# alexv879/ClusterMachineLearningForHospitalNetworks-Apache-Spark

Hardware: AMD Instinct MI355X
Metric: KMeans fit samples/sec (whole node), 100M×256 k=256 at 1/2/4/8 MI355X (higher is better)
Workload: dtype bf16; 1 GPU; model=KMeans k=256, 100000000x256, global_batch=100000000, parallelism=dp1, k=256, rows=100000000, dim=256

## Files before the change

clustermachinelearningforhospitalnetworks_apache_spark_amd/_native/csrc/kmeans.hip:

```cpp
#include <algorithm>

#include "common.h"

namespace {

constexpr int kAccumThreads = 1024;
constexpr int kSegThreads = 256;

template <int DP>
struct AssignShape {
  static constexpr int NCH = DP / 8;
  static constexpr int KS = DP >= 32 ? DP / 32 : 1;
};
constexpr int kAssignThreads = 512;

template <bool HI>
__device__ __forceinline__ unsigned f8x2_to_bf16x2(unsigned w) {
  typedef float f2 __attribute__((ext_vector_type(2)));
  const f2 v = __builtin_amdgcn_cvt_pk_f32_fp8((int)w, HI);
  return (__float_as_uint(v.x) >> 16) | (__float_as_uint(v.y) & 0xffff0000u);
}

template <int DP, bool F8>
__device__ __forceinline__ void load_x16(const void* __restrict__ Xv, long long n, long long ldx, long long row0,
// ... 1432 lines not shown
                        hist, rank, dout, rr::Ext{}, grid, g_rr_dbg, st);
  }
  if (xfp8) {
    switch (Dp) {
#define CML_ASSIGN8(DP)                                                                                          \
  case DP:                                                                                                       \
    return launch_assign<DP, true>(X, n, ldx, c, ldc, kc, kp, c_base, cnorm, xnorm, labels, best, first, last,  \
                                   cost_part, hist, rank, dout, grid, st)
      CML_ASSIGN8(64); CML_ASSIGN8(128); CML_ASSIGN8(256); CML_ASSIGN8(512);
#undef CML_ASSIGN8
      default: return (int)hipErrorInvalidValue;
    }
  }
#define CML_ASSIGN(DS, DP)                                                                                       \
  case DS:                                                                                                       \
    return launch_assign<DP, false>(X, n, ldx, c, ldc, kc, kp, c_base, cnorm, xnorm, labels, best, first, last, \
                                    cost_part, hist, rank, dout, grid, st)
  switch (Dp / 16) {
    CML_ASSIGN(1, 16); CML_ASSIGN(2, 32); CML_ASSIGN(4, 64); CML_ASSIGN(8, 128); CML_ASSIGN(16, 256);
    CML_ASSIGN(32, 512);
    default: return (int)hipErrorInvalidValue;
  }
#undef CML_ASSIGN
}

CML_API int cml_kmeans_assign_rr_ext(int mode, const void* X, long long n, long long ldx, int Dp, const void* C,
                                     long long ldc, int kc, int kp, const float* cnorm, const float* xnorm,
                                     int* labels, double* cost_part, int* hist, int* rank, int grid, int xfp8,
                                     int* chg_rows, int* chg_old, int* chg_wg_count, int* chg_overflow, int chg_pcap,
                                     int rr_ct, const int* idx, const int* n_dev, const int* lab_in, float* ub,
                                     float* lb, const float* mc, float tau, const int* gate, int want, float* best,
                                     const float* cum, int k_cum, float* mcost, int* mnear, int moff,
                                     void* stream) {
  if (mode < 1 || mode > 2 || kc != kp || kc % 16 != 0 || ldc % 8 != 0) return (int)hipErrorInvalidValue;
  if ((mcost == nullptr) != (mnear == nullptr) || (mcost != nullptr && mode != 2)) return (int)hipErrorInvalidValue;
  if (xfp8 ? (ldx % 16 != 0) : (ldx % 8 != 0)) return (int)hipErrorInvalidValue;
  if (rr_ct <= 0 || rr::plan_ct(Dp, kc, xfp8 != 0) != rr_ct) return (int)hipErrorInvalidValue;
  if (xnorm == nullptr || ub == nullptr || lb == nullptr || mc == nullptr) return (int)hipErrorInvalidValue;
  if ((hist == nullptr) != (rank == nullptr)) return (int)hipErrorInvalidValue;
  if (mode == 2 && (idx == nullptr || n_dev == nullptr || lab_in == nullptr || hist != nullptr))
    return (int)hipErrorInvalidValue;
  if (chg_rows != nullptr && (chg_old == nullptr || chg_wg_count == nullptr || chg_overflow == nullptr || chg_pcap < 0))
    return (int)hipErrorInvalidValue;
  const long long lds = rr::lds_for(Dp, kp, xfp8 != 0, mode);
  if (lds <= 0 || lds > 160 * 1024) return (int)hipErrorInvalidValue;
  const DeltaOut dout{chg_rows, chg_old, chg_wg_count, chg_overflow, chg_pcap, nullptr};
  const rr::Ext ext{idx,  n_dev, lab_in, ub,    lb,    mc,   tau, gate, want, cum, cum != nullptr ? cum + k_cum : nullptr,
                    mcost, mnear, moff};
  return rr::dispatch(mode, Dp, rr_ct, xfp8 != 0, X, n, ldx, (const u16*)C, ldc, kc, kp, cnorm, xnorm, labels,
                      best, cost_part, hist, rank, dout, ext, grid, g_rr_dbg, (hipStream_t)stream);
}

extern "C" int cml_kmeans_row_pass(const void* X, long long n, long long ldx, int Dp, int xfp8, float* xn,
                                   const float* c0, float c0n, float* cost, int* near, unsigned* xn_max,
                                   int* erange, double* xn64, const float* c0n_dev, void* stream);

CML_API int cml_row_sqnorm_fp8(const void* X, long long n, long long ldx, int Dp, float* out, void* stream) {
  return cml_kmeans_row_pass(X, n, ldx, Dp, 1, out, nullptr, 0.f, nullptr, nullptr, nullptr, nullptr, nullptr,
                             nullptr, stream);
}

CML_API int cml_row_sqnorm_bf16(const void* X, long long n, long long ldx, int Dp, float* out, void* stream) {
  return cml_kmeans_row_pass(X, n, ldx, Dp, 0, out, nullptr, 0.f, nullptr, nullptr, nullptr, nullptr, nullptr,
                             nullptr, stream);
}

CML_API long long cml_kmeans_priv_lds_bytes(int k, int dw, int rpw) { return priv_lds_bytes(k, dw, rpw); }

CML_API int cml_kmeans_accum_priv(const void* X, long long n, long long ldx, const int* labels, int k, int dw, int cpl,
                                  int rpw, float* slab, int* cslab, int gx, int nsl, void* stream) {
  hipStream_t st = (hipStream_t)stream;
// ... 174 lines not shown
```

clustermachinelearningforhospitalnetworks_apache_spark_amd/_native/csrc/kmeans_rr.h:

```cpp
#pragma once

namespace rr {

constexpr int kThreads = 512;
constexpr int kCompute = 4;

struct Ext {
  const int* idx;
  const int* n_dev;
  const int* lab_in;
  float* ub;
  float* lb;
  const float* mc;
  float tau;
  const int* gate;
  int want;
  const float* cu = nullptr;
  const float* cl = nullptr;
  float* mcost = nullptr;
  int* mnear = nullptr;
  int moff = 0;
};

__host__ __device__ constexpr int cn_slots(int kp) { return ((kp + 3) & ~3) > 256 ? ((kp + 3) & ~3) : 256; }

template <int DP, bool F8 = false, int MODE = 0, bool M32 = false>
struct Geo {
  static constexpr int KS = DP / 32;
  static constexpr int ROWB = F8 ? DP : DP * 2;
  static constexpr int TR = 32768 / ROWB;
  static constexpr int NSUB = TR / 16;
  static constexpr int SLOT = TR * ROWB;
  static constexpr int PIECES = SLOT / 1024;
  static constexpr int RPP = 1024 / ROWB;
  static constexpr int LPR = ROWB / 16;
  static constexpr int TRAIL_Q = TR >= 64 ? TR / 64 : 1;
  static constexpr int NARR = MODE == 2 ? 3 : 2;
  static constexpr int CNT0 = PIECES / 2 + TRAIL_Q;
  static constexpr int CNT1 = PIECES / 2 + (NARR - 1) * TRAIL_Q;
  static constexpr int TRB = TR * 4 * NARR;
  static constexpr int NK = MODE >= 1 ? 2 : 1;
  static constexpr int NQ = M32 ? 8 : 16;
  static constexpr int STRIDE = NQ * NK + 1;
  static constexpr int RED = TR * STRIDE * 4;
  static constexpr int LAG = M32 ? 2 : 1;
  static constexpr int NKB = LAG + 1;
  static constexpr long long fixed_bytes(int ns, int kp) {
    const long long kp4 = (kp + 3) & ~3;
    return (long long)(ns + LAG) * TRB + (long long)NKB * RED + 4LL * kp4 + (M32 ? 4LL * cn_slots(kp) : 0LL) + 64;
  }
  static constexpr int NS = (4LL * SLOT + fixed_bytes(4, 1024)) <= 160 * 1024 ? 4 : 3;
  static constexpr int NTR = NS + LAG;
};

template <int DP, bool F8 = false, int MODE = 0, bool M32 = false>
__host__ __device__ constexpr long long lds_bytes(int kp) {
  using G = Geo<DP, F8, MODE, M32>;
  return (long long)G::NS * G::SLOT + G::fixed_bytes(G::NS, kp);
}

template <int N>
__device__ __forceinline__ void wait_vm() {
  static_assert(N >= 0 && N < 64, "vmcnt field is 6 bits");
  __builtin_amdgcn_s_waitcnt((N & 15) | ((N >> 4) << 14) | (7 << 4) | (15 << 8));
}

__device__ __forceinline__ void wait_lgkm0() { asm volatile("s_waitcnt lgkmcnt(0)" ::: "memory"); }

__device__ __forceinline__ void barrier() {
  asm volatile("" ::: "memory");
  __builtin_amdgcn_s_barrier();
  asm volatile("" ::: "memory");
}

__device__ __forceinline__ void glds16(const void* src, unsigned char* lds) {
  __builtin_amdgcn_global_load_lds(src, (__attribute__((address_space(3))) void*)lds, 16, 0, 0);
}
__device__ __forceinline__ void glds4(const void* src, unsigned char* lds) {
  __builtin_amdgcn_global_load_lds(src, (__attribute__((address_space(3))) void*)lds, 4, 0, 0);
}

typedef const __attribute__((address_space(4))) int* cidx_t;

__device__ __forceinline__ int med3(int a, int b, int c) {
  const int lo = a < b ? a : b, hi = a < b ? b : a;
// ... 316 lines not shown
        }
        sc2[h] = mx_split_half(w0, w1, wh[h], wl[h]);
        __builtin_amdgcn_sched_barrier(0);
      }
      chi[ct][b] = mx_v8i{(int)wh[0][0], (int)wh[0][1], (int)wh[0][2], (int)wh[0][3],
                          (int)wh[1][0], (int)wh[1][1], (int)wh[1][2], (int)wh[1][3]};
      clo[ct][b] = mx_v8i{(int)wl[0][0], (int)wl[0][1], (int)wl[0][2], (int)wl[0][3],
                          (int)wl[1][0], (int)wl[1][1], (int)wl[1][2], (int)wl[1][3]};
      const int src = r + 16 * (2 * (g & 1));
      const int s0 = __shfl(sc2[0], src, 64);
      const int s1 = __shfl(sc2[1], src, 64);
      csc[ct][b] = (g >> 1) ? s1 : s0;
      __builtin_amdgcn_sched_barrier(0);
    }
#pragma unroll
    for (int i = 0; i < 4; ++i) {
      const int c2 = cw0 + ct * 16 + 4 * g + i;
      c4[ct][i] = c2 < kc ? cnorm[c2] : __builtin_huge_valf();
    }
  }
  __builtin_amdgcn_s_setprio(1);
  int boff[4];
#pragma unroll
  for (int b = 0; b < 4; ++b) boff[b] = r * G::ROWB + (((4 * b + g) ^ r) << 4);
  barrier();
  for (long long j = 0; j < nt; ++j) {
    if (dbg & 2) {
      wait_lgkm0();
      barrier();
      continue;
    }
    const unsigned char* xs = smem + (int)(j % G::NS) * G::SLOT;
    const float* tn = reinterpret_cast<const float*>(trail + (int)(j % G::NTR) * G::TRB);
    int* kred = red + (int)(j & 1) * G::TR * G::STRIDE;
    float xnv[G::NSUB];
#pragma unroll
    for (int t = 0; t < G::NSUB; ++t) xnv[t] = tn[16 * t + r];
    auto xaddr = [&](int u) {
      const int t = u / UPS, v = u % UPS;
      return xs + 16 * t * G::ROWB + 256 * (v >> 2) + boff[v & 3];
    };
    uint4 xr[RING];
#pragma unroll
    for (int u = 0; u < PF && u < NU; ++u) xr[u] = *reinterpret_cast<const uint4*>(xaddr(u));
    f32x4 acc[2][CT];
    int key[2] = {0x7fffffff, 0x7fffffff};
    int key2[2] = {0x7fffffff, 0x7fffffff};
#pragma unroll
    for (int u = 0; u < NU; ++u) {
      const int t = u / UPS, v = u % UPS, cur = t & 1, prv = cur ^ 1;
      if (u + PF < NU) xr[(u + PF) % RING] = *reinterpret_cast<const uint4*>(xaddr(u + PF));
      if (v & 1) {
        const int s = v >> 1;
        const uint4 a0 = xr[(u - 1) % RING], a1 = xr[u % RING];
        const mx_v8i xb = mx_v8i{(int)a0.x, (int)a0.y, (int)a0.z, (int)a0.w, (int)a1.x, (int)a1.y, (int)a1.z, (int)a1.w};
        if (s == 0) {
          key[cur] = 0x7fffffff;
          if constexpr (TOP2) key2[cur] = 0x7fffffff;
        }
#pragma unroll
        for (int ct = 0; ct < CT; ++ct) {
          const f32x4 a = __builtin_amdgcn_mfma_scale_f32_16x16x128_f8f6f4(
              chi[ct][s], xb, s == 0 ? (c4[ct] + xnv[t]) : acc[cur][ct], 0, 0, 0, csc[ct][s], 0, 127);
          acc[cur][ct] = __builtin_amdgcn_mfma_scale_f32_16x16x128_f8f6f4(clo[ct][s], xb, a, 0, 0, 1, csc[ct][s], 0, 127);
        }
        if (t > 0) {
#pragma unroll
          for (int e = (s * CT * 4) / NB; e < ((s + 1) * CT * 4) / NB; ++e) {
            const int ct = e >> 2, i = e & 3;
            const int kv = (__float_as_int(acc[prv][ct][i]) & ~TAGM) | (ct << 2 | i);
            if constexpr (TOP2) key2[prv] = med3(key[prv], kv, key2[prv]);
            key[prv] = kv < key[prv] ? kv : key[prv];
          }
          if (s == NB - 1) {
            kred[(16 * (t - 1) + r) * G::STRIDE + wave * 4 + g] = key[prv];
            if constexpr (TOP2) kred[(16 * (t - 1) + r) * G::STRIDE + 16 + wave * 4 + g] = key2[prv];
          }
        }
      }
      __builtin_amdgcn_sched_barrier(0);
    }
    {
      constexpr int t = G::NSUB - 1, cur = t & 1;
#pragma unroll
      for (int e = 0; e < CT * 4; ++e) {
        const int ct = e >> 2, i = e & 3;
        const int kv = (__float_as_int(acc[cur][ct][i]) & ~TAGM) | (ct << 2 | i);
        if constexpr (TOP2) key2[cur] = med3(key[cur], kv, key2[cur]);
        key[cur] = kv < key[cur] ? kv : key[cur];
      }
      kred[(16 * t + r) * G::STRIDE + wave * 4 + g] = key[cur];
      if constexpr (TOP2) kred[(16 * t + r) * G::STRIDE + 16 + wave * 4 + g] = key2[cur];
    }
    wait_lgkm0();
    barrier();
  }
}

template <int DP, int CT, bool F8, int MODE, bool M32, bool MX = false>
__global__ __launch_bounds__(kThreads, 1) void kmeans_assign_rr(
    const unsigned char* __restrict__ X, long long n, long long ldx, const u16* __restrict__ C, long long ldc, int kc,
    int kp, const float* __restrict__ cnorm, const float* __restrict__ xnorm, int* __restrict__ labels,
    float* __restrict__ best_out, double* __restrict__ cost_part, int* __restrict__ hist_out,
    int* __restrict__ rank_out, DeltaOut dout, Ext ext, int dbg) {
  using G = Geo<DP, F8, MODE, M32>;
  constexpr int KS = G::KS;
  constexpr int NS = G::NS;
  constexpr int CPW = CT * 16;
  constexpr int TAGB = 2 + (CT > 1) + (CT > 2) + (CT > 4);
  constexpr int TAGM = (1 << TAGB) - 1;
  constexpr bool TOP2 = MODE >= 1;
  if (ext.gate != nullptr && *ext.gate != ext.want) return;
  if constexpr (MODE == 2) n = *ext.n_dev;
  const int* lab_src = MODE == 2 ? ext.lab_in : labels;
  extern __shared__ __attribute__((aligned(16))) unsigned char smem[];
  unsigned char* trail = smem + NS * G::SLOT;
  int* red = reinterpret_cast<int*>(trail + G::NTR * G::TRB);
  int* hist = red + G::NKB * G::TR * G::STRIDE;
  float* cnl = reinterpret_cast<float*>(hist + ((kp + 3) & ~3));
  int* misc = M32 ? reinterpret_cast<int*>(cnl + cn_slots(kp)) : hist + ((kp + 3) & ~3);
  double* cost_sh = reinterpret_cast<double*>(misc + 2);

  const int tid = threadIdx.x, lane = tid & 63, wave = __builtin_amdgcn_readfirstlane(tid >> 6);
  const long long ntiles = (n + G::TR - 1) / G::TR;
  const long long nt = ntiles > blockIdx.x ? (ntiles - 1 - blockIdx.x) / gridDim.x + 1 : 0;
  const bool ranking = rank_out != nullptr;
  auto tile_of = [&](long long j) { return (long long)blockIdx.x + j * gridDim.x; };

  if (wave < kCompute) {
// ... 2 lines not shown
   } else if constexpr (M32) {
    for (int i = tid; i < cn_slots(kp); i += kCompute * 64) cnl[i] = i < kc ? cnorm[i] : __builtin_huge_valf();
    compute_m32<DP, CT, F8, MODE>(C, ldc, kc, nt, wave, lane, smem, cnl, dbg);
   } else {
    const int r = lane & 15, g = lane >> 4;
    const int cw0 = wave * CPW;
    bf16x8 creg[CT][KS];
    f32x4 c4[CT];
#pragma unroll
    for (int ct = 0; ct < CT; ++ct) {
      const int c = cw0 + ct * 16 + r;
#pragma unroll
      for (int s = 0; s < KS; ++s) {
        uint4 v = make_uint4(0u, 0u, 0u, 0u);
        const int k0 = F8 ? 64 * (s >> 1) + 16 * g + 8 * (s & 1) : 32 * s + 8 * g;
        if (c < kc) v = *reinterpret_cast<const uint4*>(C + (long long)c * ldc + k0);
        const unsigned w4[4] = {v.x, v.y, v.z, v.w};
        unsigned o[4];
#pragma unroll
        for (int e = 0; e < 4; ++e) {
          const float lo = -2.f * bf16_to_f32((u16)(w4[e] & 0xffffu));
          const float hi = -2.f * bf16_to_f32((u16)(w4[e] >> 16));
          o[e] = (unsigned)f32_to_bf16(lo) | ((unsigned)f32_to_bf16(hi) << 16);
        }
        creg[ct][s] = __builtin_bit_cast(bf16x8, make_uint4(o[0], o[1], o[2], o[3]));
      }
#pragma unroll
      for (int i = 0; i < 4; ++i) {
        const int c2 = cw0 + ct * 16 + 4 * g + i;
        c4[ct][i] = c2 < kc ? cnorm[c2] : __builtin_huge_valf();
      }
    }
    __builtin_amdgcn_s_setprio(1);
    int boff[4];
#pragma unroll
    for (int b = 0; b < 4; ++b) boff[b] = r * G::ROWB + (((4 * b + g) ^ r) << 4);
    barrier();
    for (long long j = 0; j < nt; ++j) {
      if (dbg & 2) {
        wait_lgkm0();
        barrier();
        continue;
      }
      const unsigned char* xs = smem + (int)(j % NS) * G::SLOT;
      const float* tn = reinterpret_cast<const float*>(trail + (int)(j % G::NTR) * G::TRB);
      int* kred = red + (int)(j & 1) * G::TR * G::STRIDE;
      constexpr int SPU = F8 ? 2 : 1;
      constexpr int UPS = KS / SPU;
      constexpr int NU = G::NSUB * UPS;
      constexpr int PF = 3;
      float xnv[G::NSUB];
#pragma unroll
      for (int t = 0; t < G::NSUB; ++t) xnv[t] = tn[16 * t + r];
      auto xaddr = [&](int u) {
        const int t = u / UPS, v = u % UPS;
        return xs + 16 * t * G::ROWB + 256 * (v >> 2) + boff[v & 3];
      };
      uint4 xr[PF + 1];
#pragma unroll
      for (int u = 0; u < PF && u < NU; ++u) xr[u] = *reinterpret_cast<const uint4*>(xaddr(u));
      f32x4 acc[2][CT];
      int key[2] = {0x7fffffff, 0x7fffffff};
      int key2[2] = {0x7fffffff, 0x7fffffff};
#pragma unroll
      for (int u = 0; u < NU; ++u) {
        const int t = u / UPS, v = u % UPS, cur = t & 1, prv = cur ^ 1;
        if (u + PF < NU) xr[(u + PF) % (PF + 1)] = *reinterpret_cast<const uint4*>(xaddr(u + PF));
        bf16x8 xb[SPU];
        if constexpr (F8) {
          const uint4 w = xr[u % (PF + 1)];
          const unsigned ws[4] = {w.x, w.y, w.z, w.w};
          unsigned o[8];
#pragma unroll
          for (int q = 0; q < 4; ++q) {
            o[2 * q] = __builtin_bit_cast(unsigned, __builtin_amdgcn_cvt_scalef32_pk_bf16_fp8(ws[q], 1.0f, false));
            o[2 * q + 1] = __builtin_bit_cast(unsigned, __builtin_amdgcn_cvt_scalef32_pk_bf16_fp8(ws[q], 1.0f, true));
          }
          xb[0] = __builtin_bit_cast(bf16x8, make_uint4(o[0], o[1], o[2], o[3]));
          xb[SPU - 1] = __builtin_bit_cast(bf16x8, make_uint4(o[4], o[5], o[6], o[7]));
        } else {
          xb[0] = __builtin_bit_cast(bf16x8, xr[u % (PF + 1)]);
        }
#pragma unroll
        for (int h = 0; h < SPU; ++h) {
          const int s = v * SPU + h;
          if (s == 0) {
            key[cur] = 0x7fffffff;
            if constexpr (TOP2) key2[cur] = 0x7fffffff;
          }
#pragma unroll
          for (int ct = 0; ct < CT; ++ct)
            acc[cur][ct] = __builtin_amdgcn_mfma_f32_16x16x32_bf16(
                creg[ct][s], xb[h], s == 0 ? (c4[ct] + xnv[t]) : acc[cur][ct], 0, 0, 0);
          if (t > 0) {
#pragma unroll
            for (int e = (s * CT * 4) / KS; e < ((s + 1) * CT * 4) / KS; ++e) {
              const int ct = e >> 2, i = e & 3;
              const int kv = (__float_as_int(acc[prv][ct][i]) & ~TAGM) | (ct << 2 | i);
              if constexpr (TOP2) key2[prv] = med3(key[prv], kv, key2[prv]);
              key[prv] = kv < key[prv] ? kv : key[prv];
            }
            if (s == KS - 1) {
              kred[(16 * (t - 1) + r) * G::STRIDE + wave * 4 + g] = key[prv];
              if constexpr (TOP2) kred[(16 * (t - 1) + r) * G::STRIDE + 16 + wave * 4 + g] = key2[prv];
            }
          }
        }
        __builtin_amdgcn_sched_barrier(0);
      }
      {
        constexpr int t = G::NSUB - 1, cur = t & 1;
#pragma unroll
        for (int e = 0; e < CT * 4; ++e) {
          const int ct = e >> 2, i = e & 3;
          const int kv = (__float_as_int(acc[cur][ct][i]) & ~TAGM) | (ct << 2 | i);
          if constexpr (TOP2) key2[cur] = med3(key[cur], kv, key2[cur]);
          key[cur] = kv < key[cur] ? kv : key[cur];
        }
        kred[(16 * t + r) * G::STRIDE + wave * 4 + g] = key[cur];
        if constexpr (TOP2) kred[(16 * t + r) * G::STRIDE + 16 + wave * 4 + g] = key2[cur];
      }
      wait_lgkm0();
      barrier();
    }
   }
  } else if (wave < kCompute + 2) {
    const int dw = wave - kCompute;
    for (long long j = 0; j < NS - 1 && j < nt && !(dbg & 1); ++j)
      issue_tile<DP, F8, MODE, M32>(X, ldx, n, xnorm, lab_src, ext.idx, tile_of(j), (int)j, (int)j, dw, lane, smem);
    if (nt >= NS - 1) {
      if (dw == 0) wait_vm<(NS - 2) * G::CNT0>();
      else wait_vm<(NS - 2) * G::CNT1>();
    } else {
      wait_vm<0>();
    }
    barrier();
    for (long long j = 0; j < nt; ++j) {
      const long long jn = j + NS - 1;
      if (jn < nt && !(dbg & 1)) {
        issue_tile<DP, F8, MODE, M32>(X, ldx, n, xnorm, lab_src, ext.idx, tile_of(jn), (int)(jn % NS),
                                      (int)(jn % G::NTR), dw, lane, smem);
        if (dw == 0) wait_vm<(NS - 2) * G::CNT0>();
        else wait_vm<(NS - 2) * G::CNT1>();
      } else {
        wait_vm<0>();
      }
      barrier();
    }
    if constexpr (M32) barrier();
  } else {
    const int fw = wave - kCompute - 2;
    constexpr int RPF = G::TR / 2;
    if (fw == 0) {
      for (int i = lane; i < kp; i += 64) hist[i] = 0;
      if (lane == 0) misc[0] = 0;
    }
    double cost = 0.0;
    float mcv = 0.f;
    if constexpr (TOP2) mcv = *ext.mc;
    constexpr int LPR_F = 64 / RPF;
    constexpr int QPL = G::NQ / LPR_F;
    const int rl = lane % RPF, part = lane / RPF;
    auto finalize = [&](long long j) {
      const int* kr = red + (int)(j % G::NKB) * G::TR * G::STRIDE;
      const unsigned char* te = trail + (int)(j % G::NTR) * G::TRB;
      const int R = fw * RPF + rl;
      const long long pos = tile_of(j) * G::TR + R;
      int kv[QPL], kv2[QPL];
#pragma unroll
      for (int q = 0; q < QPL; ++q) {
        kv[q] = kr[R * G::STRIDE + part * QPL + q];
        if constexpr (TOP2) kv2[q] = kr[R * G::STRIDE + G::NQ + part * QPL + q];
      }
      const int old = reinterpret_cast<const int*>(te + G::TR * 4)[R];
      long long row = pos;
      if constexpr (MODE == 2) row = reinterpret_cast<const int*>(te + G::TR * 8)[R];
      unsigned long long best = ~0ull;
      unsigned sec = ~0u;
#pragma unroll
      for (int q = 0; q < QPL; ++q) {
        const int qq = part * QPL + q;
        unsigned idx;
// ... 22 lines not shown
        const unsigned long long ob = __shfl_xor(best, o, 64);
        if constexpr (TOP2) {
          const unsigned os = __shfl_xor(sec, o, 64);
          const unsigned bv = (unsigned)(best >> 32), obv = (unsigned)(ob >> 32);
          const unsigned mx = obv > bv ? obv : bv;
          const unsigned s2 = os < sec ? os : sec;
          sec = mx < s2 ? mx : s2;
        }
        best = ob < best ? ob : best;
      }
      const int bi = (int)(best & 0xffffffffu);
      const float dist = fmaxf(__int_as_float((int)((unsigned)(best >> 32) ^ 0x80000000u)), 0.f);
      const bool mine = part == 0 && pos < n;
      const bool ch = mine && old != bi;
      if (dout.rows != nullptr) {
        const unsigned long long bal = __ballot(ch);
        if (bal != 0ull) {
          const int leader = __builtin_ctzll(bal);
          int base = 0;
          if (lane == leader) base = atomicAdd(misc, (int)__popcll(bal));
          base = __shfl(base, leader, 64);
          const int at = base + (int)__popcll(bal & ((1ull << lane) - 1ull));
          if (ch && at < dout.pcap) {
            const long long o = (long long)blockIdx.x * dout.pcap + at;
            dout.rows[o] = (int)row;
            dout.old[o] = old;
          }
        }
      }
      if (ch) labels[row] = bi;
      if (mine) {
        cost += (double)dist;
        if (best_out != nullptr) best_out[row] = dist;
        if constexpr (MODE == 2) {
          if (ext.mcost != nullptr && dist < ext.mcost[row]) {
            ext.mcost[row] = dist;
            ext.mnear[row] = bi + ext.moff;
          }
        }
        if (ranking) rank_out[row] = atomicAdd(hist + bi, 1);
        if constexpr (TOP2) {
          const float xn = reinterpret_cast<const float*>(te)[R];
          const float slack = ext.tau * (xn + mcv);
          const float sd = __int_as_float((int)(sec ^ 0x80000000u));
          float u = sqrtf(dist + slack) * (1.0f + 1e-6f);
          float w = sqrtf(fmaxf(sd - slack, 0.f)) * (1.0f - 1e-6f);
          if (ext.cu != nullptr) {
            const float cu = ext.cu[bi], cl = ext.cl[bi];
            u = (u - cu) + 1e-6f * (u + cu);
            w = (w + cl) - 1e-6f * (w + cl);
          }
          ext.ub[row] = u;
          ext.lb[row] = w;
        }
      }
    };
    wait_lgkm0();
    barrier();
    constexpr int LAG = G::LAG;
    for (long long j = 0; j < nt; ++j) {
      if (j >= LAG && !(dbg & 4)) finalize(j - LAG);
      wait_lgkm0();
      barrier();
    }
    if constexpr (LAG == 2) {
      if (nt >= 2 && !(dbg & 4)) finalize(nt - 2);
      wait_lgkm0();
// ... 44 lines not shown
      case 512: return lds_bytes<512, true, MODE, M32>(kp);
      default: return 0;
    }
  }
  switch (Dp) {
    case 128: return lds_bytes<128, false, MODE, M32>(kp);
    case 256: return lds_bytes<256, false, MODE, M32>(kp);
    case 512: return lds_bytes<512, false, MODE, M32>(kp);
    default: return 0;
  }
}

inline long long lds_for(int Dp, int kp, bool f8 = false, int mode = 0) {
  const bool m32 = use_m32(Dp, plan_ct(Dp, kp, f8), f8);
  switch (mode * 2 + (m32 ? 1 : 0)) {
    case 0: return lds_for_mode<0, false>(Dp, kp, f8);
    case 1: return lds_for_mode<0, true>(Dp, kp, f8);
    case 2: return lds_for_mode<1, false>(Dp, kp, f8);
    case 3: return lds_for_mode<1, true>(Dp, kp, f8);
    case 4: return lds_for_mode<2, false>(Dp, kp, f8);
    case 5: return lds_for_mode<2, true>(Dp, kp, f8);
    default: return 0;
  }
}

inline int g_mx = 1;
inline bool use_mx(int Dp, bool f8, bool m32) { return f8 && g_mx && !m32 && Dp % 128 == 0; }

template <int DP, int CT, bool F8, int MODE, bool M32, bool MX = false>
int launch(const void* X, long long n, long long ldx, const u16* C, long long ldc, int kc, int kp, const float* cnorm,
           const float* xnorm, int* labels, float* best, double* cost_part, int* hist, int* rank, DeltaOut dout,
           Ext ext, int grid, int dbg, hipStream_t st) {
  const size_t lds = (size_t)lds_bytes<DP, F8, MODE, M32>(kp);
  if (lds > 160 * 1024) return (int)hipErrorInvalidValue;
  const void* fn = (const void*)kmeans_assign_rr<DP, CT, F8, MODE, M32, MX>;
  hipFuncSetAttribute(fn, hipFuncAttributeMaxDynamicSharedMemorySize, (int)lds);
  const long long ldb = F8 ? ldx : 2 * ldx;
  hipLaunchKernelGGL((kmeans_assign_rr<DP, CT, F8, MODE, M32, MX>), dim3(grid), dim3(kThreads), lds, st,
                     (const unsigned char*)X, n, ldb, C, ldc, kc, kp, cnorm, xnorm, labels, best, cost_part, hist,
                     rank, dout, ext, dbg);
  return cml_status();
}

template <int MODE>
inline int dispatch_mode(int Dp, int ct, bool f8, const void* X, long long n, long long ldx, const u16* C,
                         long long ldc, int kc, int kp, const float* cnorm, const float* xnorm, int* labels,
                         float* best, double* cost_part, int* hist, int* rank, DeltaOut dout, Ext ext, int grid,
                         int dbg, hipStream_t st) {
  const bool m32 = use_m32(Dp, ct, f8);
  if (use_mx(Dp, f8, m32)) {
#define CML_RX(D, T)                                                                                                \
  if (Dp == D && ct == T)                                                                                           \
  return launch<D, T, true, MODE, false, true>(X, n, ldx, C, ldc, kc, kp, cnorm, xnorm, labels, best, cost_part,   \
                                               hist, rank, dout, ext, grid, dbg, st)
    CML_RX(256, 1); CML_RX(256, 2); CML_RX(256, 3); CML_RX(256, 4);
    CML_RX(512, 1); CML_RX(512, 2);
#undef CML_RX
    return (int)hipErrorInvalidValue;
  }
#define CML_RR(D, T, F, M)                                                                                          \
  if (Dp == D && ct == T && f8 == F && m32 == M)                                                                    \
  return launch<D, T, F, MODE, M>(X, n, ldx, C, ldc, kc, kp, cnorm, xnorm, labels, best, cost_part, hist, rank,    \
                                  dout, ext, grid, dbg, st)
  CML_RR(128, 1, false, false); CML_RR(128, 2, false, false); CML_RR(128, 3, false, false);
  CML_RR(128, 4, false, false); CML_RR(128, 5, false, false);
  CML_RR(256, 1, false, false); CML_RR(256, 2, false, false); CML_RR(256, 3, false, false);
  CML_RR(256, 4, false, false); CML_RR(256, 5, false, false);
// ... 28 lines not shown
```

clustermachinelearningforhospitalnetworks_apache_spark_amd/models/kmeans.py:

```python
from __future__ import annotations

import math
import os
import types
from typing import List, Optional

import numpy as np
import torch

from .. import _native
from ..ops import kmeans_ops as K
from ..ops.group_ops import group_reduce
from ..parallel.comm import Communicator, local_comm
from ..utils import rng
from ..utils.device import padded_dim, round_up
from ..utils.fault import maybe_fail
from ..utils.trace import trace


def padded_dim_fp8(d: int) -> int:
    return max(256, 1 << max(0, (d - 1).bit_length()))


def to_device_matrix(x: torch.Tensor, d: Optional[int] = None) -> torch.Tensor:
# ... 1740 lines not shown
        nearest = alloc(max(n, 1), dtype=torch.int32, device=dev)
        self._row_pass(cb0[0].to(torch.float32).contiguous(), 0.0, costs, nearest, c0n_dev=cn0[0:1])
        return costs, nearest

    def _init_scratch(self):
        sc = self._iscr
        if sc is None:
            n, dev = self.n, self.device
            tr = self.aplan.round_rows
            sc = types.SimpleNamespace()
            sc.lab = torch.empty(max(n, 1), dtype=torch.int32, device=dev)
            sc.best = torch.empty(max(n, 1), dtype=torch.float32, device=dev)
            sc.list_a = torch.empty((max(n, 1), 4), dtype=torch.int32, device=dev)
            sc.list_b = torch.zeros(n + tr, dtype=torch.int32, device=dev)
            sc.cxn = torch.zeros(n + tr, dtype=torch.float32, device=dev)
            sc.lab_in = torch.full((n + tr,), -1, dtype=torch.int32, device=dev)
            sc.cnt = torch.zeros(2, dtype=torch.int32, device=dev)
            self._iscr = sc
        return sc

    def _init_candidate_pass(self, m: int, cbn: torch.Tensor, cnn: torch.Tensor, c_off: int, costs: torch.Tensor,
                             nearest: torch.Tensor, off: int) -> None:
        n, dp, dev = self.n, self.dp, self.device
        if n == 0:
            return
        sc = self._init_scratch()
        lab, best = sc.lab[:n], sc.best[:n]
        xn = self.xnorm
        parts, c0 = [], 0
        for size in self._candidate_chunks(m):
            kp = round_up(size, 32)
            parts.append((c0, size, cbn[c_off + c0:c_off + c0 + kp], cnn[c_off + c0:c_off + c0 + kp]))
            c0 += size
        for _, r0, r1, xc in self._x_chunks(whole=True):
            mm = r1 - r0
            if mm == 0:
                continue
            for c0, kc, cb, cn in parts:
                plan = K.plan_assign(mm, dp, kc, dev.index or 0, fp8=K.is_fp8(self.x))
                K.assign_bf16(xc, mm, dp, cb, cn, plan, lab[r0:r1], best[r0:r1], None, xnorm=xn[r0:r1])
                K.init_merge(costs[r0:r1], nearest[r0:r1], best[r0:r1], lab[r0:r1], off + c0, mm)

    _INIT_LMAX = 8

    def _init_candidate_pass_pruned(self, prev: torch.Tensor, new: torch.Tensor, cbn: torch.Tensor,
                                    cnn: torch.Tensor, c_off: int, costs: torch.Tensor, nearest: torch.Tensor,
                                    off: int) -> bool:
        n, d, dp, dev = self.n, self.d, self.dp, self.device
        mode = os.environ.get("CML_KMEANS_INIT_PRUNE", "auto")
        if mode == "0" or (mode == "auto" and dp > 256):
            return False
        if not self._pdev or not self._rr_max_chunk():
            return False
        if n == 0:
            return True
        m = int(new.shape[0])
        tab = K.init_table(prev, new)
        if tab is not None:
            tab_v, tab_j, pn32 = tab
        else:
            P = prev.to(device=dev, dtype=torch.float64)
            Y = new.to(device=dev, dtype=torch.float64)
            pn, yn = (P * P).sum(1), (Y * Y).sum(1)
            d2 = pn[:, None] + yn[None, :] - 2.0 * (P @ Y.T)
            eps = 1e-12 * (pn.max() + yn.max())
            vals, order = torch.sort((d2 - eps).clamp_(min=0.0).sqrt_().mul_(1.0 - 1e-6), dim=1)
            tab_v = vals.to(torch.float32).contiguous()
            tab_j = order.to(torch.int32).contiguous()
            pn32 = (pn * (1.0 + 1e-6)).to(torch.float32).contiguous()
        tau = 2.0 * self._tau
        sc = self._init_scratch()
        list_a, list_b, cnt = sc.list_a, sc.list_b, sc.cnt
# ... 92 lines not shown
```

clustermachinelearningforhospitalnetworks_apache_spark_amd/ops/kmeans_ops.py:

```python
from __future__ import annotations

import ctypes
import os
import threading

from dataclasses import dataclass

import torch

from .. import _native
from .._native import c_dbl, c_int, c_ll, c_vp
from ..utils.device import LDS_BUDGET, num_cus, round_up

_native.register_kernel_sigs({
    "cml_kmeans_assign_lds_bytes": (c_ll, [c_int, c_int, c_int]),
    "cml_kmeans_assign_threads": (c_int, [c_int]),
    "cml_kmeans_set_assign_variant": (c_int, [c_int]),
    "cml_kmeans_assign_occupancy": (c_int, [c_int, c_int, c_int, c_int]),
    "cml_kmeans_seg_threads": (c_int, []),
    "cml_kmeans_seg_ints": (c_ll, [c_int]),
    "cml_kmeans_assign_bf16": (c_int, [c_vp, c_ll, c_ll, c_int, c_vp, c_ll, c_int, c_int, c_int, c_vp, c_vp, c_vp,
                                       c_vp, c_int, c_int, c_vp, c_vp, c_vp, c_int, c_int, c_vp, c_vp, c_vp, c_vp,
                                       c_int, c_int, c_vp]),
    "cml_kmeans_assign_rr_plan": (c_int, [c_int, c_int, c_int, c_int, c_vp]),
# ... 841 lines not shown
    _apply_env_knobs(lib)
    return bool(lib.cml_kmeans_set_fp8_mx(-1))


def mx_applies(x: torch.Tensor) -> bool:
    return x.is_cuda and is_fp8(x) and fp8_mx_on()


def assign_rr_ext(mode: int, x: torch.Tensor, n: int, dp: int, cb: torch.Tensor, cnorm: torch.Tensor,
                  plan: AssignPlan, xnorm: torch.Tensor, labels: torch.Tensor, cost_part: torch.Tensor | None,
                  ub: torch.Tensor, lb: torch.Tensor, mc: torch.Tensor, tau: float,
                  hist: torch.Tensor | None = None, rank: torch.Tensor | None = None,
                  delta: "DeltaState | None" = None, idx: torch.Tensor | None = None,
                  n_dev: torch.Tensor | None = None, lab_in: torch.Tensor | None = None,
                  gate: torch.Tensor | None = None, want: int = 0, stream=None,
                  best: torch.Tensor | None = None, cum: torch.Tensor | None = None,
                  merge_cost: torch.Tensor | None = None, merge_near: torch.Tensor | None = None,
                  merge_off: int = 0) -> None:
    if plan.rr_ct <= 0 or plan.kc != plan.kp:
        raise ValueError("the pruned-step assign needs the K9r plan (Dp in {128, 256, 512}, k <= 256)")
    _native.check(_native.kernels().cml_kmeans_assign_rr_ext(
        int(mode), x.data_ptr(), int(n), x.stride(0), int(dp), cb.data_ptr(), cb.stride(0), plan.kc, plan.kp,
        cnorm.data_ptr(), xnorm.data_ptr(), labels.data_ptr(), _ptr(cost_part), _ptr(hist), _ptr(rank),
        plan.grid, int(is_fp8(x)),
        _ptr(delta.rows if delta is not None else None), _ptr(delta.old if delta is not None else None),
        _ptr(delta.wg_count if delta is not None else None), _ptr(delta.overflow if delta is not None else None),
        delta.pcap if delta is not None else 0, plan.rr_ct, _ptr(idx), _ptr(n_dev), _ptr(lab_in), ub.data_ptr(),
        lb.data_ptr(), mc.data_ptr(), float(tau), _ptr(gate), int(want), _ptr(best), _ptr(cum),
        int(cum.shape[0] // 2) if cum is not None else 0, _ptr(merge_cost), _ptr(merge_near), int(merge_off),
        _native.stream_ptr(stream)),
        f"kmeans_assign_rr_ext(mode={mode})")


def init_classify(cost: torch.Tensor, near: torch.Tensor, xn: torch.Tensor, pn: torch.Tensor, tab_v: torch.Tensor,
                  tau: float, n: int, lmax: int, list_a: torch.Tensor, cnt_a: torch.Tensor, list_b: torch.Tensor,
                  cnt_b: torch.Tensor, stream=None) -> None:
    if list_a.dtype != torch.int32 or list_a.numel() < 4 * n:
        raise ValueError("list_a: int32 [n, 4] entries")
    m = int(tab_v.shape[1])
    _native.check(_native.kernels().cml_kmeans_init_classify(
        cost.data_ptr(), near.data_ptr(), xn.data_ptr(), pn.data_ptr(), tab_v.data_ptr(), m, float(tau), int(n),
        int(lmax), list_a.data_ptr(), cnt_a.data_ptr(), list_b.data_ptr(), cnt_b.data_ptr(),
        _native.stream_ptr(stream)), "kmeans_init_classify")


def unique_rows(P: torch.Tensor):
    if not P.is_cuda or P.dim() != 2 or P.shape[0] == 0 or P.shape[0] > 8192:
        return torch.unique(P, dim=0, return_inverse=True)
    P = P.to(torch.float64).contiguous()
    m, d = int(P.shape[0]), int(P.shape[1])
    dup = torch.empty(m, dtype=torch.int32, device=P.device)
    inv = torch.empty(m, dtype=torch.int64, device=P.device)
    uniq = torch.empty((m, d), dtype=torch.float64, device=P.device)
    count = torch.zeros(1, dtype=torch.int32, device=P.device)
    _native.check(_native.kernels().cml_kmeans_unique_rows(P.data_ptr(), m, d, dup.data_ptr(), inv.data_ptr(),
                                                           uniq.data_ptr(), count.data_ptr(), _native.stream_ptr()),
                  "kmeans_unique_rows")
    return uniq[: int(count.item())], inv


def init_table(P: torch.Tensor, Y: torch.Tensor, stream=None):
    mp, d = int(P.shape[0]), int(P.shape[1])
    m = int(Y.shape[0])
    if m > 1024 or not P.is_cuda:
        return None
    P = P.to(torch.float64).contiguous()
# ... 368 lines not shown
```

Baseline: 111.4 billion samples/s.

## Fuse init candidate merge into RR assign and carry last sub-tile keys across steps

Adds a mode-0 path to the K9r assign kernel that writes the min-cost/nearest merge directly, so the k-means++ init loop no longer runs a separate assign followed by an init_merge pass. In the compute waves, the key reduction for the final sub-tile is deferred into the next step's MFMA stream (LAG=2 with a third reduction buffer) so it overlaps with matrix work instead of stalling at the tail. The LDS layout is re-derived for a 320-centroid cap, and xnorm loads are staggered. This costs extra LDS for the additional reduction buffer, a trailing barrier and flush, and more complex indexing.

Measured after the change: 111.7 billion samples/s (median of 2 runs). About the same (+0.2%).

```diff
diff --git a/clustermachinelearningforhospitalnetworks_apache_spark_amd/_native/csrc/kmeans.hip b/clustermachinelearningforhospitalnetworks_apache_spark_amd/_native/csrc/kmeans.hip
--- a/clustermachinelearningforhospitalnetworks_apache_spark_amd/_native/csrc/kmeans.hip
+++ b/clustermachinelearningforhospitalnetworks_apache_spark_amd/_native/csrc/kmeans.hip
@@ -1488,11 +1488,13 @@
                                      float* lb, const float* mc, float tau, const int* gate, int want, float* best,
                                      const float* cum, int k_cum, float* mcost, int* mnear, int moff,
                                      void* stream) {
-  if (mode < 1 || mode > 2 || kc != kp || kc % 16 != 0 || ldc % 8 != 0) return (int)hipErrorInvalidValue;
-  if ((mcost == nullptr) != (mnear == nullptr) || (mcost != nullptr && mode != 2)) return (int)hipErrorInvalidValue;
+  if (mode < 0 || mode > 2 || kc != kp || kc % 16 != 0 || ldc % 8 != 0) return (int)hipErrorInvalidValue;
+  if ((mcost == nullptr) != (mnear == nullptr) || (mcost != nullptr && mode == 1)) return (int)hipErrorInvalidValue;
+  if (mode == 0 && mcost == nullptr) return (int)hipErrorInvalidValue;
   if (xfp8 ? (ldx % 16 != 0) : (ldx % 8 != 0)) return (int)hipErrorInvalidValue;
   if (rr_ct <= 0 || rr::plan_ct(Dp, kc, xfp8 != 0) != rr_ct) return (int)hipErrorInvalidValue;
-  if (xnorm == nullptr || ub == nullptr || lb == nullptr || mc == nullptr) return (int)hipErrorInvalidValue;
+  if (xnorm == nullptr) return (int)hipErrorInvalidValue;
+  if (mode >= 1 && (ub == nullptr || lb == nullptr || mc == nullptr)) return (int)hipErrorInvalidValue;
   if ((hist == nullptr) != (rank == nullptr)) return (int)hipErrorInvalidValue;
   if (mode == 2 && (idx == nullptr || n_dev == nullptr || lab_in == nullptr || hist != nullptr))
     return (int)hipErrorInvalidValue;
diff --git a/clustermachinelearningforhospitalnetworks_apache_spark_amd/_native/csrc/kmeans_rr.h b/clustermachinelearningforhospitalnetworks_apache_spark_amd/_native/csrc/kmeans_rr.h
--- a/clustermachinelearningforhospitalnetworks_apache_spark_amd/_native/csrc/kmeans_rr.h
+++ b/clustermachinelearningforhospitalnetworks_apache_spark_amd/_native/csrc/kmeans_rr.h
@@ -21,6 +21,9 @@
   int* mnear = nullptr;
   int moff = 0;
 };
+
+constexpr int kMaxK = 320;
+constexpr long long kLdsMax = 160 * 1024;
 
 __host__ __device__ constexpr int cn_slots(int kp) { return ((kp + 3) & ~3) > 256 ? ((kp + 3) & ~3) : 256; }
 
@@ -43,14 +46,17 @@
   static constexpr int NQ = M32 ? 8 : 16;
   static constexpr int STRIDE = NQ * NK + 1;
   static constexpr int RED = TR * STRIDE * 4;
-  static constexpr int LAG = M32 ? 2 : 1;
+  static constexpr long long fixed_for(int lag, int ns, int kp) {
+    const long long kp4 = (kp + 3) & ~3;
+    return (long long)(ns + lag) * TRB + (long long)(lag + 1) * RED + 4LL * kp4 + (M32 ? 4LL * cn_slots(kp) : 0LL) + 64;
+  }
+  static constexpr int ns_for(int lag) { return 4LL * SLOT + fixed_for(lag, 4, kMaxK) <= kLdsMax ? 4 : 3; }
+  static constexpr int LAG = M32 || (MODE == 0 && ns_for(2) == ns_for(1)) ? 2 : 1;
   static constexpr int NKB = LAG + 1;
-  static constexpr long long fixed_bytes(int ns, int kp) {
-    const long long kp4 = (kp + 3) & ~3;
-    return (long long)(ns + LAG) * TRB + (long long)NKB * RED + 4LL * kp4 + (M32 ? 4LL * cn_slots(kp) : 0LL) + 64;
-  }
-  static constexpr int NS = (4LL * SLOT + fixed_bytes(4, 1024)) <= 160 * 1024 ? 4 : 3;
+  static constexpr long long fixed_bytes(int ns, int kp) { return fixed_for(LAG, ns, kp); }
+  static constexpr int NS = ns_for(LAG);
   static constexpr int NTR = NS + LAG;
+  static_assert((long long)NS * SLOT + fixed_bytes(NS, kMaxK) <= kLdsMax, "K9r LDS layout exceeds 160 KiB");
 };
 
 template <int DP, bool F8 = false, int MODE = 0, bool M32 = false>
@@ -433,7 +439,7 @@
     }
     const unsigned char* xs = smem + (int)(j % G::NS) * G::SLOT;
     const float* tn = reinterpret_cast<const float*>(trail + (int)(j % G::NTR) * G::TRB);
-    int* kred = red + (int)(j & 1) * G::TR * G::STRIDE;
+    int* kred = red + (int)(j % G::NKB) * G::TR * G::STRIDE;
     float xnv[G::NSUB];
 #pragma unroll
     for (int t = 0; t < G::NSUB; ++t) xnv[t] = tn[16 * t + r];
@@ -496,6 +502,7 @@
     wait_lgkm0();
     barrier();
   }
+  if constexpr (G::LAG == 2) barrier();
 }
 
 template <int DP, int CT, bool F8, int MODE, bool M32, bool MX = false>
@@ -564,9 +571,37 @@
       }
     }
     __builtin_amdgcn_s_setprio(1);
-    int boff[4];
-#pragma unroll
-    for (int b = 0; b < 4; ++b) boff[b] = r * G::ROWB + (((4 * b + g) ^ r) << 4);
+    const int boff0 = r * G::ROWB + ((g ^ r) << 4);
+    static_assert(G::ROWB % 256 == 0 && G::SLOT % 256 == 0, "B fragment offsets: bits 6-7 are the step's");
+    constexpr bool CARRY = G::LAG == 2;
+    constexpr int SPU = F8 ? 2 : 1;
+    constexpr int UPS = KS / SPU;
+    constexpr int NU = G::NSUB * UPS;
+    constexpr int PF = 3;
+    constexpr int KSP = KS >= 8 ? KS - 1 : KS;
+    constexpr int NE = CT * 4;
+    static_assert(G::NSUB % 2 == 0, "the carried sub-tile sits in accumulator set 1");
+    f32x4 acc[2][CT];
+    int key[2] = {0x7fffffff, 0x7fffffff};
+    int key2[2] = {0x7fffffff, 0x7fffffff};
+    if constexpr (CARRY) {
+#pragma unroll
+      for (int ct = 0; ct < CT; ++ct) acc[1][ct] = f32x4{0.f, 0.f, 0.f, 0.f};
+    }
+    auto keys = [&](int p, int e0, int e1) {
+#pragma unroll
+      for (int e = e0; e < e1; ++e) {
+        const int ct = e >> 2, i = e & 3;
+        const int kv = (__float_as_int(acc[p][ct][i]) & ~TAGM) | (ct << 2 | i);
+        if constexpr (TOP2) key2[p] = med3(key[p], kv, key2[p]);
+        key[p] = kv < key[p] ? kv : key[p];
+      }
+    };
+    auto put_keys = [&](int* kd, int p, int row) {
+      kd[row * G::STRIDE + wave * 4 + g] = key[p];
+      if constexpr (TOP2) kd[row * G::STRIDE + 16 + wave * 4 + g] = key2[p];
+    };
+    int sx = 0, st = 0, sk = 0;
     barrier();
     for (long long j = 0; j < nt; ++j) {
       if (dbg & 2) {
@@ -574,30 +609,27 @@
         barrier();
         continue;
       }
-      const unsigned char* xs = smem + (int)(j % NS) * G::SLOT;
-      const float* tn = reinterpret_cast<const float*>(trail + (int)(j % G::NTR) * G::TRB);
-      int* kred = red + (int)(j & 1) * G::TR * G::STRIDE;
-      constexpr int SPU = F8 ? 2 : 1;
-      constexpr int UPS = KS / SPU;
-      constexpr int NU = G::NSUB * UPS;
-      constexpr int PF = 3;
-      float xnv[G::NSUB];
-#pragma unroll
-      for (int t = 0; t < G::NSUB; ++t) xnv[t] = tn[16 * t + r];
+      const int xs = sx * G::SLOT + boff0;
+      const float* tn = reinterpret_cast<const float*>(trail + st * G::TRB);
+      int* kred = red + sk * G::TR * G::STRIDE;
+      int* kprev = red + (sk == 0 ? G::NKB - 1 : sk - 1) * G::TR * G::STRIDE;
+      sx = sx + 1 == NS ? 0 : sx + 1;
+      st = st + 1 == G::NTR ? 0 : st + 1;
+      sk = sk + 1 == G::NKB ? 0 : sk + 1;
       auto xaddr = [&](int u) {
         const int t = u / UPS, v = u % UPS;
-        return xs + 16 * t * G::ROWB + 256 * (v >> 2) + boff[v & 3];
+        return smem + (xs ^ ((v & 3) << 6)) + 16 * t * G::ROWB + 256 * (v >> 2);
       };
+      float xnv[G::NSUB];
+      xnv[0] = tn[r];
       uint4 xr[PF + 1];
 #pragma unroll
       for (int u = 0; u < PF && u < NU; ++u) xr[u] = *reinterpret_cast<const uint4*>(xaddr(u));
-      f32x4 acc[2][CT];
-      int key[2] = {0x7fffffff, 0x7fffffff};
-      int key2[2] = {0x7fffffff, 0x7fffffff};
 #pragma unroll
       for (int u = 0; u < NU; ++u) {
         const int t = u / UPS, v = u % UPS, cur = t & 1, prv = cur ^ 1;
         if (u + PF < NU) xr[(u + PF) % (PF + 1)] = *reinterpret_cast<const uint4*>(xaddr(u + PF));
+        if (v == 0 && t + 1 < G::NSUB) xnv[t + 1] = tn[16 * (t + 1) + r];
         bf16x8 xb[SPU];
         if constexpr (F8) {
           const uint4 w = xr[u % (PF + 1)];
@@ -624,33 +656,27 @@
           for (int ct = 0; ct < CT; ++ct)
             acc[cur][ct] = __builtin_amdgcn_mfma_f32_16x16x32_bf16(
                 creg[ct][s], xb[h], s == 0 ? (c4[ct] + xnv[t]) : acc[cur][ct], 0, 0, 0);
-          if (t > 0) {
-#pragma unroll
-            for (int e = (s * CT * 4) / KS; e < ((s + 1) * CT * 4) / KS; ++e) {
-              const int ct = e >> 2, i = e & 3;
-              const int kv = (__float_as_int(acc[prv][ct][i]) & ~TAGM) | (ct << 2 | i);
-              if constexpr (TOP2) key2[prv] = med3(key[prv], kv, key2[prv]);
-              key[prv] = kv < key[prv] ? kv : key[prv];
-            }
-            if (s == KS - 1) {
-              kred[(16 * (t - 1) + r) * G::STRIDE + wave * 4 + g] = key[prv];
-              if constexpr (TOP2) kred[(16 * (t - 1) + r) * G::STRIDE + 16 + wave * 4 + g] = key2[prv];
+          if (s < KSP && (t > 0 || CARRY)) {
+            keys(prv, (s * NE) / KSP, ((s + 1) * NE) / KSP);
+            if (s == KSP - 1) {
+              if (t > 0) put_keys(kred, prv, 16 * (t - 1) + r);
+              else put_keys(kprev, prv, 16 * (G::NSUB - 1) + r);
             }
           }
         }
         __builtin_amdgcn_sched_barrier(0);
       }
-      {
-        constexpr int t = G::NSUB - 1, cur = t & 1;
-#pragma unroll
-        for (int e = 0; e < CT * 4; ++e) {
-          const int ct = e >> 2, i = e & 3;
-          const int kv = (__float_as_int(acc[cur][ct][i]) & ~TAGM) | (ct << 2 | i);
-          if constexpr (TOP2) key2[cur] = med3(key[cur], kv, key2[cur]);
-          key[cur] = kv < key[cur] ? kv : key[cur];
-        }
-        kred[(16 * t + r) * G::STRIDE + wave * 4 + g] = key[cur];
-        if constexpr (TOP2) kred[(16 * t + r) * G::STRIDE + 16 + wave * 4 + g] = key2[cur];
+      if constexpr (!CARRY) {
+        keys(1, 0, NE);
+        put_keys(kred, 1, 16 * (G::NSUB - 1) + r);
+      }
+      wait_lgkm0();
+      barrier();
+    }
+    if constexpr (CARRY) {
+      if (nt > 0 && !(dbg & 2)) {
+        keys(1, 0, NE);
+        put_keys(red + (sk == 0 ? G::NKB - 1 : sk - 1) * G::TR * G::STRIDE, 1, 16 * (G::NSUB - 1) + r);
       }
       wait_lgkm0();
       barrier();
@@ -679,7 +705,7 @@
       }
       barrier();
     }
-    if constexpr (M32) barrier();
+    if constexpr (G::LAG == 2) barrier();
   } else {
     const int fw = wave - kCompute - 2;
     constexpr int RPF = G::TR / 2;
@@ -768,7 +794,7 @@
       if (mine) {
         cost += (double)dist;
         if (best_out != nullptr) best_out[row] = dist;
-        if constexpr (MODE == 2) {
+        if constexpr (MODE != 1) {
           if (ext.mcost != nullptr && dist < ext.mcost[row]) {
             ext.mcost[row] = dist;
             ext.mnear[row] = bi + ext.moff;
@@ -879,7 +905,7 @@
            const float* xnorm, int* labels, float* best, double* cost_part, int* hist, int* rank, DeltaOut dout,
            Ext ext, int grid, int dbg, hipStream_t st) {
   const size_t lds = (size_t)lds_bytes<DP, F8, MODE, M32>(kp);
-  if (lds > 160 * 1024) return (int)hipErrorInvalidValue;
+  if (kp > kMaxK || lds > (size_t)kLdsMax) return (int)hipErrorInvalidValue;
   const void* fn = (const void*)kmeans_assign_rr<DP, CT, F8, MODE, M32, MX>;
   hipFuncSetAttribute(fn, hipFuncAttributeMaxDynamicSharedMemorySize, (int)lds);
   const long long ldb = F8 ? ldx : 2 * ldx;
diff --git a/clustermachinelearningforhospitalnetworks_apache_spark_amd/models/kmeans.py b/clustermachinelearningforhospitalnetworks_apache_spark_amd/models/kmeans.py
--- a/clustermachinelearningforhospitalnetworks_apache_spark_amd/models/kmeans.py
+++ b/clustermachinelearningforhospitalnetworks_apache_spark_amd/models/kmeans.py
@@ -1796,12 +1796,17 @@
             kp = round_up(size, 32)
             parts.append((c0, size, cbn[c_off + c0:c_off + c0 + kp], cnn[c_off + c0:c_off + c0 + kp]))
             c0 += size
+        fold = self._hs is None and os.environ.get("CML_KMEANS_INIT_FOLD", "1") != "0"
         for _, r0, r1, xc in self._x_chunks(whole=True):
             mm = r1 - r0
             if mm == 0:
                 continue
             for c0, kc, cb, cn in parts:
                 plan = K.plan_assign(mm, dp, kc, dev.index or 0, fp8=K.is_fp8(self.x))
+                if fold and plan.rr_ct > 0 and plan.kc == plan.kp:
+                    K.assign_rr_merge(xc, mm, dp, cb, cn, plan, xn[r0:r1], lab[r0:r1], costs[r0:r1],
+                                      nearest[r0:r1], off + c0)
+                    continue
                 K.assign_bf16(xc, mm, dp, cb, cn, plan, lab[r0:r1], best[r0:r1], None, xnorm=xn[r0:r1])
                 K.init_merge(costs[r0:r1], nearest[r0:r1], best[r0:r1], lab[r0:r1], off + c0, mm)
 
diff --git a/clustermachinelearningforhospitalnetworks_apache_spark_amd/ops/kmeans_ops.py b/clustermachinelearningforhospitalnetworks_apache_spark_amd/ops/kmeans_ops.py
--- a/clustermachinelearningforhospitalnetworks_apache_spark_amd/ops/kmeans_ops.py
+++ b/clustermachinelearningforhospitalnetworks_apache_spark_amd/ops/kmeans_ops.py
@@ -897,6 +897,18 @@
         f"kmeans_assign_rr_ext(mode={mode})")
 
 
+def assign_rr_merge(x: torch.Tensor, n: int, dp: int, cb: torch.Tensor, cnorm: torch.Tensor, plan: AssignPlan,
+                    xnorm: torch.Tensor, labels: torch.Tensor, merge_cost: torch.Tensor, merge_near: torch.Tensor,
+                    merge_off: int, stream=None) -> None:
+    if plan.rr_ct <= 0 or plan.kc != plan.kp:
+        raise ValueError("the fused candidate merge needs the K9r plan")
+    _native.check(_native.kernels().cml_kmeans_assign_rr_ext(
+        0, x.data_ptr(), int(n), x.stride(0), int(dp), cb.data_ptr(), cb.stride(0), plan.kc, plan.kp,
+        cnorm.data_ptr(), xnorm.data_ptr(), labels.data_ptr(), 0, 0, 0, plan.grid, int(is_fp8(x)), 0, 0, 0, 0, 0,
+        plan.rr_ct, 0, 0, 0, 0, 0, 0, 0.0, 0, 0, 0, 0, 0, merge_cost.data_ptr(), merge_near.data_ptr(),
+        int(merge_off), _native.stream_ptr(stream)), "kmeans_assign_rr_ext(mode=0, merge)")
+
+
 def init_classify(cost: torch.Tensor, near: torch.Tensor, xn: torch.Tensor, pn: torch.Tensor, tab_v: torch.Tensor,
                   tau: float, n: int, lmax: int, list_a: torch.Tensor, cnt_a: torch.Tensor, list_b: torch.Tensor,
                   cnt_b: torch.Tensor, stream=None) -> None:
```
